# EDIpack/EDIpack

Measured on AMD Instinct MI355X. Metric: Lanczos H*v iterations/sec, largest (Nup,Ndw) sector, higher is better.
Workload: dtype f64

## Files before the change

edipack_amd/capi.py:

```python
from __future__ import annotations

import ctypes as C
import os

import numpy as np

HERE = os.path.dirname(os.path.abspath(__file__))
LIB_PATH = os.environ.get("EDIGPU_LIB", os.path.join(HERE, "lib", "libedigpu.so"))
HEADER_PATH = os.path.join(os.path.dirname(HERE), "include", "edigpu.h")

MAXORB = 5
MAXSUNDRY = 64
MAXBATH = 16


class EdigpuError(RuntimeError):
    """Raised when a C-ABI call returns non-zero (the Fortran shim does ``stop msg``)."""


class EdigpuModel(C.Structure):
    _fields_ = [
        ("ed_mode", C.c_int32), ("bath_type", C.c_int32),
        ("norb", C.c_int32), ("nbath", C.c_int32), ("nspin", C.c_int32), ("hfmode", C.c_int32),
        ("xmu", C.c_double),
# ... 90 lines not shown
    "edigpu_imp_rdm": (C.c_int, [_vp, _vp, C.c_int, _pd, _pd]),
    "edigpu_time_rdm": (C.c_int, [_vp, _vp, C.c_int, C.c_int, _pd]),
    "edigpu_imp_rdm_flat": (C.c_int, [_vp, _vp, C.c_int, _pd, _pd]),
    "edigpu_time_rdm_flat": (C.c_int, [_vp, _vp, C.c_int, C.c_int, _pd]),
    "edigpu_apply_xph": (C.c_int, [_vp, _vp, _vp, _vp]),
    "edigpu_ph_rdm": (C.c_int, [_vp, _vp, C.c_int, _pd, _pd]),
    "edigpu_time_ph": (C.c_int, [_vp, _vp, _vp, C.c_int, C.c_int, _pd]),
    "edigpu_pairs_sector": (C.c_int, [C.POINTER(EdigpuModel), C.c_int, C.c_int, C.c_int, _pi32, _pi32, _pi32, _pi32, _pi32,
                                      _pi32, _pint, _pint, _pint]),
    "edigpu_apply_pairs_normal": (C.c_int, [_vp, _vp, _vp, _vp, C.c_int, _pd, _pi32, _pi32, _pi32, _pi32, _pi32, _pi32, _vp]),
    "edigpu_time_pairs": (C.c_int, [_vp, _vp, _vp, _vp, C.c_int, _pd, _pi32, _pi32, _pi32, _pi32, _pi32, _pi32, C.c_int,
                                    C.c_int, _pd]),
    "edigpu_vec_work_doubles": (C.c_int, []),
    "edigpu_vec_rotate": (C.c_int, [_i64, _vp, _vp, _vp, _vp]),
    "edigpu_vec_add_dot": (C.c_int, [_i64, _vp, _vp, _vp, _vp, _vp, _vp]),
    "edigpu_vec_axpy_nrm2": (C.c_int, [_i64, _vp, _vp, _vp, _vp, _vp, _vp]),
    "edigpu_vec_scale": (C.c_int, [_i64, _vp, _vp, _vp]),
    "edigpu_vec_rotate_lazy": (C.c_int, [_i64, _vp, _vp, _vp, _vp]),
    "edigpu_vec_add_dot2": (C.c_int, [_i64, _vp, _vp, _vp, _vp, _vp, _vp]),
    "edigpu_time_apply": (C.c_int, [_vp, C.c_int, C.c_int, C.c_int, _pd]),
    "edigpu_lanczos_bench": (C.c_int, [_vp, C.c_int, C.c_int, _pd, _pd]),
    "edigpu_apply_loop_d": (C.c_int, [_vp, _i64, _pd, _pd]),
    "edigpu_tile_task_map": (C.c_int, [C.c_int32, C.c_int32, C.c_int32, _pi32, _pi32, _pi32, _pi32, _pi32]),
    "edigpu_ell16_images": (C.c_int, [_i64, _pi64, _pi32, _pd, _pi64, _vp, _vp, _pi64]),
    "edigpu_finalize_ab": (C.c_int, [C.c_int32, _pd, _i64, _pd, _pd, C.c_int32, _pd, C.c_int32, C.c_int32]),
    "edigpu_trl_dots": (C.c_int, [C.c_int32, _i64, C.c_int32, _pd, C.c_int32, _i64, _i64, _pd, _i64, C.c_int32, _pd, _i64,
                                  C.c_int32]),
    "edigpu_trl_norm2": (C.c_int, [C.c_int32, _i64, _pd, _i64, _pd, _i64]),
    "edigpu_trl_subtract": (C.c_int, [C.c_int32, _i64, C.c_int32, _pd, C.c_int32, _i64, _i64, _pd, _i64, _pd, _i64,
                                      C.c_int32]),
    "edigpu_trl_decide": (C.c_int, [_pd, _i64, C.c_int32, C.c_double, C.c_double, _pd, _i64, _pi32]),
    "edigpu_trl_filter": (C.c_int, [_pd, _i64, C.c_int32, C.c_double]),
    "edigpu_trl_rotate": (C.c_int, [_i64, C.c_int32, C.c_int32, _pd, _i64, _i64, _pd, C.c_int32, _i64, _pd, _i64, _i64]),
    "edigpu_trl_scale": (C.c_int, [_i64, _pd, _i64, C.c_double]),
    "edigpu_membw": (C.c_int, [_i64, _pd]),
    "edigpu_sector_map": (C.c_int, [_vp, C.c_int, C.c_int, C.c_int, _pi32, _pi64]),
    "edigpu_cache_create": (C.c_int, [C.POINTER(_vp), _i64]),
    "edigpu_cache_get": (C.c_int, [_vp, C.POINTER(EdigpuModel), C.c_int, C.c_int, C.c_int, C.POINTER(_vp)]),
    "edigpu_cache_stats": (C.c_int, [_vp, _pi64]),
    "edigpu_cache_clear": (C.c_int, [_vp]),
    "edigpu_cache_destroy": (C.c_int, [_vp]),
    "edigpu_dev_alloc": (C.c_int, [_i64, C.POINTER(_vp)]),
    "edigpu_dev_free": (C.c_int, [_vp]),
    "edigpu_dev_upload": (C.c_int, [_vp, _vp, _i64]),
    "edigpu_dev_download": (C.c_int, [_vp, _vp, _i64]),
    "edigpu_shard_plan": (C.c_int, [_i64, C.c_int32, C.c_int32, _pi64, _pi64, _pi64]),
# ... 90 lines not shown
```

edipack_amd/csrc/edigpu_capi.hip:

```cpp
#include <algorithm>
#include <map>
#include <mutex>
#include <tuple>

#include "dev_mem.hpp"
#include "host_ib.hpp"
#include "kernels.hpp"

namespace edigpu {

static thread_local std::string g_err;
static thread_local int g_device = 0;
void set_error(const std::string& msg) { g_err = msg; }

bool have_error() { return !g_err.empty(); }
int current_device() { return g_device; }

int ensure_device(int* count_out) {
  int n = 0;
  hipError_t e = hipGetDeviceCount(&n);
  if (e != hipSuccess || n <= 0) {
    set_error(std::string("edigpu: no usable HIP device (") +
              (e != hipSuccess ? hipGetErrorString(e) : "device count 0") +
              "); this library has no CPU fallback");
// ... 242 lines not shown
  if (bytes > 0) EDIGPU_HIP(hipMemcpy(dst_dev, src_host, (size_t)bytes, hipMemcpyHostToDevice));
  return 0;
}

int edigpu_dev_download(void* dst_host, const void* src_dev, int64_t bytes) {
  if (bytes < 0 || (bytes > 0 && (!dst_host || !src_dev))) {
    set_error("edigpu_dev_download: bad argument");
    return 1;
  }
  if (bytes > 0) EDIGPU_HIP(hipMemcpy(dst_host, src_dev, (size_t)bytes, hipMemcpyDeviceToHost));
  return 0;
}

int edigpu_destroy(edigpu_handle s) {
  if (!s) return 0;
  (void)hipSetDevice(s->device);
  if (s->stream) {
    (void)hipStreamSynchronize(s->stream);
    (void)hipStreamDestroy(s->stream);
  }
  if (s->sub_s) edigpu_destroy(s->sub_s);
  if (s->sub_a) edigpu_destroy(s->sub_a);
  if (s->sub_d) edigpu_destroy(s->sub_d);
  dev_free_all(s->d_cz, s->d_hd, s->d_gu, s->d_gd, s->d_mx_rowptr, s->d_tile_chunks, s->d_tile_lbeg);
  if (s->lz_graph) (void)hipGraphExecDestroy(s->lz_graph);
  dev_free_all(s->d_lzcnt, s->d_bl_meta, s->d_bl_lend, s->d_bl_ent, s->d_bl_wtab);
  if (s->ib) {
    free_ib(s->ib);
    delete s->ib;
    s->ib = nullptr;
  }
  dev_free_all(s->d_tl_meta, s->d_tl_col, s->d_tl_val, s->d_mx_col, s->d_mx_val);
  dev_free_all(s->d_eux, s->d_ed, s->d_impd, s->d_ndcoef, s->d_jup, s->d_jdw);
  free_ell(s->up_ell);
  free_csr(s->dw);
  free_csr(s->nd);
  free_csr(s->loc);
  free_csr(s->nonloc);
  dev_free_all(s->orbs.ell_col, s->orbs.ell_val, s->orbs.hd, s->orbs.eax, s->orbs.impbit, s->orbs.xtab);
  s->orbs = OrbsArgs();
  dev_free_all(s->d_dir_states, s->d_dir_offdw, s->d_dir_rkup, s->d_dir_terms, s->d_dir_tests, s->d_dir_dtab, s->d_dir_xtab);
  free_occ(s);
  free_rdm(s);
  free_rdm_flat(s);
  free_ph(s);
  free_axisop(s);
  free_batch(s);
// ... 7 lines not shown
```

edipack_amd/csrc/edigpu_internal.hpp:

```cpp
#pragma once
#include <hip/hip_runtime.h>

#include <cstdint>
#include <cstdio>
#include <functional>
#include <memory>
#include <string>
#include <vector>

#include "../../include/edigpu.h"
#include "host_build.hpp"
#include "switches.hpp"

namespace edigpu {

enum SectorKind : int { kNormal = 0, kFlat = 1, kDirect = 2, kOrbs = 3, kCmplxNormal = 4 };

void set_error(const std::string& msg);
#pragma GCC visibility push(hidden)
bool have_error();
int current_device();
int ensure_device(int* count_out = nullptr);
#pragma GCC visibility pop

// ... 178 lines not shown
  double* d_hd = nullptr;
  edigpu::DevEll up_ell;
  edigpu::DevCsr dw;
  int dw_maxrow = 0;
  edigpu::DevCsr nd;
  int has_nd = 0;
  edigpu::HostCsr h_up, h_dw;
  int rows_per_block = 1;
  int factored = 0;
  int fac_nimp = 0, fac_nterms = 0;
  double* d_eux = nullptr;
  double* d_ed = nullptr;
  uint8_t* d_impd = nullptr;
  double* d_ndcoef = nullptr;
  uint32_t* d_jup = nullptr;
  edigpu_sector* sub_s = nullptr;
  edigpu_sector* sub_a = nullptr;
  edigpu_sector* sub_d = nullptr;
  double* d_cz = nullptr;
  int panel_mode = 0;
  int tile_nchunks = 0, tile_rows = 0;
  int32_t* d_tile_chunks = nullptr;
  int32_t* d_tile_lbeg = nullptr;
  int tile_list_cap = 0;
  int4* d_tl_meta = nullptr;
  int32_t* d_tl_col = nullptr;
  double* d_tl_val = nullptr;
  int tl_has_nd = 0;
  int blk_shift = 0;
  int blk_tail_balance = 1;
  int64_t blk_ps = 0, blk_len = 0;
  int4* d_bl_meta = nullptr;
  int blk_rows = 0;
  int blk_list_cap = 0;
  int32_t* d_bl_lend = nullptr;
  uint32_t* d_bl_ent = nullptr;
  double* d_bl_wtab = nullptr;
  bool lz_blocked = false;
  int64_t lz_len = 0;
  edigpu::IbDev* ib = nullptr;
  int row_split = 1;
  int col_halo = 0;
  uint32_t* d_jdw = nullptr;
  int32_t* d_mx_rowptr = nullptr;
  int32_t* d_mx_col = nullptr;
  double* d_mx_val = nullptr;
// ... 97 lines not shown
```

edipack_amd/csrc/edigpu_setup.hip:

```cpp
#include <algorithm>
#include <cstddef>
#include <memory>

#include "dev_mem.hpp"
#include "host_ib.hpp"
#include "host_pack.hpp"
#include "host_sb.hpp"
#include "kernels.hpp"

namespace edigpu {

static const int4* as_int4(const std::vector<HostInt4>& v) {
  static_assert(sizeof(HostInt4) == sizeof(int4) && offsetof(HostInt4, x) == offsetof(int4, x) &&
                    offsetof(HostInt4, y) == offsetof(int4, y) && offsetof(HostInt4, z) == offsetof(int4, z) &&
                    offsetof(HostInt4, w) == offsetof(int4, w),
                "HostInt4 is uploaded as int4");
  return reinterpret_cast<const int4*>(v.data());
}

static int upload_csr(DevCsr& d, int64_t nrow, const int64_t* rowptr, const int32_t* col,
                      const double* val, int cplx) {
  d = DevCsr();
  d.nrow = nrow;
  d.nnz = rowptr ? rowptr[nrow] : 0;
// ... 398 lines not shown
        if (dev_upload(&s->d_mx_rowptr, m.rowptr.data(), m.rowptr.size()) || dev_upload(&s->d_mx_col, m.col.data(), m.col.size()) ||
            dev_upload(&s->d_mx_val, m.val.data(), m.val.size()))
          return 1;
      }
    }
    s->h_hd = std::move(built->hd);
    s->h_nd = std::move(built->nd);
  } else {
    if (dev_upload(&s->d_hd, hd, (size_t)s->nloc)) return 1;
    if (s->has_nd && upload_csr(s->nd, s->nloc, nd_rowptr, nd_col, nd_val, 0)) return 1;
    if (s->has_nd && !sw.nd_in_rows &&
        upload_sell(s->nd, s->nloc, dim_up * dim_dw, nd_rowptr, nd_col, nd_val, 0, false, sw, 16.0))
      return 1;
  }
  if (s->panel_mode == 2) {
    const HostFactored* f = (s->factored && built) ? &built->fac : nullptr;
    const bool with_nd = f && f->nterms > 0 && s->d_mx_rowptr != nullptr;
    const HostTileLists l = build_tile_lists(dw, dim_dw, dw_first, dw_count, tile_starts, with_nd ? f : nullptr);
    s->tile_list_cap = l.list_cap;
    const std::vector<HostInt4> meta = tile_meta_live(l, dw_first);
    if (dev_upload(&s->d_tile_lbeg, l.lbeg.data(), l.lbeg.size()) || dev_upload(&s->d_tl_meta, as_int4(meta), meta.size()) ||
        dev_upload(&s->d_tl_col, l.col.data(), l.col.size()) || dev_upload(&s->d_tl_val, l.val.data(), l.val.size()))
      return 1;
    s->tl_has_nd = l.has_nd ? 1 : 0;
  }
  if (s->factored && built && built->norb > 0 && dw_first == 0 && dw_count == dim_dw) {
    const int64_t min_rows = sw.ib_min;
    bool pairs = false;
    for (int sp = 0; sp < 2 && !pairs; sp++) {
      const std::vector<double>& a = built->ob_a[sp];
      const int ns = built->ns;
      if ((int)a.size() == ns * ns)
        for (int p = built->norb; p < ns && !pairs; p++)
          for (int q = p + 1; q < ns; q++)
            if (a[(size_t)p * ns + q] != 0.0) {
              pairs = true;
              break;
            }
    }
    const bool pairs_ok = !pairs || min_rows == 0 || sw.ib_pairs;
    const bool short_rows = dim_up * 8 < sw.ib_min_row_bytes();
    if (sw.ib && pairs_ok && s->nloc >= min_rows && (!short_rows || sw.posrows) && !sw.lanczos_unfused && setup_ib(s, *built))
      return 1;
    if (s->ib && short_rows && !s->ib->pr.on) {
      free_ib(s->ib);
      delete s->ib;
// ... 244 lines not shown
```

edipack_amd/csrc/hooks/image_hooks.hip:

```cpp
#include <algorithm>
#include <climits>

#include "../dev_mem.hpp"
#include "../host_pack.hpp"
#include "../kernels.hpp"
#include "../tile_map.hpp"

using namespace edigpu;

extern "C" {

int edigpu_tile_task_map(int32_t npanels, int32_t blocks_per_panel, int32_t balanced, int32_t* grid, int32_t* np,
                         int32_t* panel, int32_t* chunk, int32_t* pos) {
  if (npanels < 1 || blocks_per_panel < 1 || !grid || !np ||
      ((int64_t)npanels + 7) / 8 * 8 * (int64_t)blocks_per_panel > INT32_MAX) {
    set_error("edigpu_tile_task_map: bad argument");
    return 1;
  }
  const TileMap m = plan_tile_map(npanels, blocks_per_panel, balanced != 0);
  *grid = m.grid;
  *np = m.np;
  for (int wg = 0; wg < m.grid; wg++) {
    int pn, ch, ps;
    if (!tile_task_of(m, npanels, blocks_per_panel, wg, pn, ch, ps)) pn = -1;
    if (panel) panel[wg] = pn;
    if (chunk) chunk[wg] = ch;
    if (pos) pos[wg] = ps;
  }
  return 0;
}

int edigpu_ell16_images(int64_t nrow, const int64_t* rowptr, const int32_t* col, const double* val, int64_t* info,
                        uint32_t* pk16, uint32_t* pk16o, int64_t* owned_col) {
  if (nrow < 1 || !rowptr || !info || (rowptr[nrow] > 0 && (!col || !val))) {
    set_error("edigpu_ell16_images: bad argument");
    return 1;
  }
  HostCsr a;
  a.nrow = a.ncol = nrow;
  a.rowptr.assign(rowptr, rowptr + nrow + 1);
  a.col.assign(col, col + rowptr[nrow]);
  a.val.assign(val, val + rowptr[nrow]);
  const HostEll h = encode_ell(a, true, true, true);
  info[0] = h.width;
  info[1] = h.pitch;
  info[2] = h.pitch16o;
  info[3] = (int64_t)h.pk16.size();
  info[4] = (int64_t)h.pk16o.size();
  if (pk16) std::copy(h.pk16.begin(), h.pk16.end(), pk16);
  if (pk16o) std::copy(h.pk16o.begin(), h.pk16o.end(), pk16o);
  if (owned_col)
// ... 31 lines not shown
```

edipack_amd/csrc/host_pack.cpp:

```cpp
#include "host_pack.hpp"

#include <algorithm>
#include <cmath>
#include <cstdlib>
#include <cstring>

namespace edigpu {

HostEll encode_ell(const HostCsr& a, bool lds, bool allow_typed, bool allow_16) {
  HostEll e;
  const uint32_t cmul = lds ? 8u : 1u;
  e.nrow = a.nrow;
  e.pitch = (a.nrow + 63) / 64 * 64;
  int w = 0;
  for (int64_t i = 0; i < a.nrow; i++) w = std::max<int>(w, (int)(a.rowptr[i + 1] - a.rowptr[i]));
  e.width = w;
  if (w == 0 || a.nrow == 0) return e;
  std::vector<double> coef(1, 0.0);
  bool packable = (a.nrow + 1) * (int64_t)cmul < ((int64_t)1 << 24);
  std::vector<uint8_t> cid((size_t)a.nnz());
  for (int64_t p = 0; p < a.nnz() && packable; p++) {
    const double m = std::fabs(a.val[p]);
    size_t k = 0;
    for (; k < coef.size(); k++)
// ... 302 lines not shown
  }
  for (size_t ch = 0; ch + 1 < tile_starts.size(); ch++) lbeg.push_back(meta[(size_t)tile_starts[ch]].x);
  lbeg.push_back((int32_t)tc.size());
  l.list_cap = 4;
  for (size_t ch = 0; ch + 1 < lbeg.size(); ch++) l.list_cap = std::max(l.list_cap, lbeg[ch + 1] - lbeg[ch]);
  tc.resize(tc.size() + 8, 0);
  tv.resize(tv.size() + 8, 0.0);
  l.has_nd = with_nd;
  return l;
}

std::vector<HostInt4> tile_meta_live(const HostTileLists& l, int64_t dw_first) {
  std::vector<HostInt4> meta = l.meta;
  for (size_t r = 0; r < meta.size(); r++) {
    HostInt4& m = meta[r];
    const int ob = m.x + m.y;
    while (m.z % 4 != 1 && m.z > 0 && l.val[(size_t)(ob + m.z - 1)] == 0.0 &&
           l.col[(size_t)(ob + m.z - 1)] == (int32_t)(dw_first + (int64_t)r))
      m.z--;
  }
  return meta;
}

HostBlockLists build_block_lists(const HostCsr& dw, const HostFactored& f, int64_t dim_dw, int shift, int64_t lds_kb) {
  HostBlockLists b;
  std::vector<double> wtab{0.0};
  auto widx = [&](double w) -> int {
    for (size_t i = 0; i < wtab.size(); i++)
      if (wtab[i] == w && std::signbit(wtab[i]) == std::signbit(w)) return (int)i;
    wtab.push_back(w);
    return (int)wtab.size() - 1;
  };
  int64_t R = std::max<int64_t>(32, std::min<int64_t>(lds_kb * 1024 / ((int64_t)8 << shift), 4096) / 32 * 32);
  std::vector<HostInt4> meta((size_t)dim_dw);
  std::vector<uint32_t> ent;
  ent.reserve((size_t)dw.rowptr[dim_dw] + 8 * (size_t)dim_dw);
  bool fits = true;
  for (int64_t g = 0; g < dim_dw && fits; g++) {
    const int64_t cs = g / R * R;
    HostInt4 m = {(int)ent.size(), 0, 0, 0};
    for (int pass = 0; pass < 2; pass++) {
      int& cnt = pass == 0 ? m.y : m.z;
      for (int64_t q = dw.rowptr[g]; q < dw.rowptr[g + 1]; q++) {
        const int64_t c = dw.col[q];
        const bool inside = c >= cs && c < cs + R;
        if (inside != (pass == 0)) continue;
// ... 51 lines not shown
```

edipack_amd/csrc/host_pack.hpp:

```cpp
#pragma once
#include <cstdint>
#include <vector>

#include "host_build.hpp"

namespace edigpu {

struct HostInt4 {
  int32_t x, y, z, w;
};

struct HostEll {
  int64_t nrow = 0, pitch = 0;
  int width = 0;
  int typed = 0;
  std::vector<uint32_t> pk;
  std::vector<double> coef;
  std::vector<uint32_t> pk16;
  std::vector<uint32_t> pk16o;
  int64_t pitch16o = 0;
  std::vector<int32_t> col;
  std::vector<double> val;
};
inline int64_t ell16_owned_col(int64_t pos) {
// ... 16 lines not shown
                     bool is_loc, double max_pad, bool allow_packed);

void plan_tile_chunks(const HostCsr& dw, int64_t dw_first, int64_t dw_count, int rmax, std::vector<int32_t>& starts,
                      int& longest);

struct HostMergedList {
  std::vector<int32_t> rowptr, col;
  std::vector<double> val;
};
HostMergedList merge_dw_lists(const HostCsr& dw, const HostFactored& f, int64_t dw_first, int64_t dw_count, int64_t dim_dw);

struct HostTileLists {
  std::vector<HostInt4> meta;
  std::vector<int32_t> col;
  std::vector<double> val;
  std::vector<int32_t> lbeg;
  int list_cap = 4;
  bool has_nd = false;
};
HostTileLists build_tile_lists(const HostCsr& dw, int64_t dim_dw, int64_t dw_first, int64_t dw_count,
                               const std::vector<int32_t>& tile_starts, const HostFactored* f);
std::vector<HostInt4> tile_meta_live(const HostTileLists& l, int64_t dw_first);

struct HostBlockLists {
  bool fits = false;
  int rows = 0;
  std::vector<HostInt4> meta;
  std::vector<uint32_t> ent;
  std::vector<double> wtab;
  std::vector<int32_t> lend;
  int list_cap = 4;
};
HostBlockLists build_block_lists(const HostCsr& dw, const HostFactored& f, int64_t dim_dw, int shift, int64_t lds_kb);

int factored_col_halo(const HostFactored& f, int64_t dim_up);

}
```

edipack_amd/csrc/kernels_normal.hip:

```cpp
#include <cstdlib>
#include <string>
#include <type_traits>

#include "kernels.hpp"
#include "normal_args.hpp"

namespace edigpu {



constexpr int kE = 4;

template <bool VEC>
__device__ inline void load4(const double* __restrict__ base, int64_t i0, const bool* ok, double* out, int64_t dB = 2) {
  if (VEC) {
    const double2 a = ok[0] ? *reinterpret_cast<const double2*>(base + i0) : make_double2(0.0, 0.0);
    const double2 b = ok[2] ? *reinterpret_cast<const double2*>(base + i0 + dB) : make_double2(0.0, 0.0);
    out[0] = a.x;
    out[1] = a.y;
    out[2] = b.x;
    out[3] = b.y;
  } else {
#pragma unroll
    for (int e = 0; e < kE; e++) out[e] = ok[e] ? base[i0 + e] : 0.0;
// ... 522 lines not shown
  a.ell_val = s->up_ell.val;
  a.ell_w = s->up_ell.width;
  a.ell_typed = s->up_ell.typed;
  a.ell_pitch = s->up_ell.pitch;
  a.ell_pitch16 = s->up_ell.pitch16;
  a.dw_rowptr = s->dw.rowptr32;
  a.dw_col = s->dw.col;
  a.dw_val = s->dw.val;
  a.dw_maxrow = s->dw_maxrow;
  a.nd_rp32 = s->nd.rowptr32;
  a.nd_rp64 = s->nd.wide ? s->nd.rowptr64 : nullptr;
  a.nd_col = s->nd.col;
  a.nd_val = s->nd.val;
  a.has_nd = s->has_nd;
  a.nterms = s->factored ? s->fac_nterms : 0;
  a.nd_coef = s->d_ndcoef;
  a.jup = s->d_jup;
  a.jdw = s->d_jdw;
  a.panel_mode = s->panel_mode;
  a.tile_nchunks = s->tile_nchunks;
  a.tile_rows = s->tile_rows;
  a.tile_chunks = s->d_tile_chunks;
  a.tile_lbeg = s->d_tile_lbeg;
  a.tile_list_cap = s->tile_list_cap;
  a.tl_meta = s->d_tl_meta;
  a.tl_col = s->d_tl_col;
  a.tl_val = s->d_tl_val;
  a.tl_has_nd = s->tl_has_nd;
  a.blk_shift = 0;
  a.blk_ps = 0;
  a.blk_tail_balance = s->blk_tail_balance;
  a.bl_meta = s->d_bl_meta;
  a.blk_rows = s->blk_rows;
  a.blk_list_cap = s->blk_list_cap;
  a.bl_lend = s->d_bl_lend;
  a.bl_ent = s->d_bl_ent;
  a.bl_wtab = s->d_bl_wtab;
  a.mx_rowptr = s->d_mx_rowptr;
  a.mx_col = s->d_mx_col;
  a.mx_val = s->d_mx_val;
  a.scal = nullptr;
  a.partial = nullptr;
  a.xout = nullptr;
  a.partial_cap = 0;
  a.lz_counter = nullptr;
  a.lz_nlanc = 0;
// ... 146 lines not shown
```

edipack_amd/csrc/kernels_panel.hip:

```cpp
#include <algorithm>
#include <cstdio>
#include <cstdlib>
#include <vector>

#include "lz_finalize.hpp"
#include "normal_args.hpp"
#include "tile_map.hpp"

namespace edigpu {

struct PanelArgs {
  int npanels, width, blocks_per_panel, rows_per_block;
  int64_t col_first, ncol, stride;
  int halo;
  int tile_rows;
  int list_cap;
  TileMap map;
};

constexpr int kPanelNT = 512;
constexpr int kMaxNdTerms = 16;

template <bool DO_DW, bool DO_ND, bool ALPHA, bool COLS = false>
__global__ void __launch_bounds__(kPanelNT)
    normal_dw_panel_kernel(NormalArgs a, PanelArgs p, const double* __restrict__ v_full,
                           double* __restrict__ hv) {
  __shared__ double red[3 * (kPanelNT / 64)];
// ... 314 lines not shown
    if (threadIdx.x == 0) {
#pragma unroll
      for (int i = 0; i < kPanelNT / 64; i++) {
        t += red[i];
        q += red[kPanelNT / 64 + i];
        n += red[2 * (kPanelNT / 64) + i];
      }
      if (!a.lz_counter) {
        a.partial[blockIdx.x] = t;
        a.partial[gridDim.x + blockIdx.x] = q;
        a.partial[2 * gridDim.x + blockIdx.x] = n;
      }
    }
    if (a.lz_counter)
      lz_finalize_if_last<kPanelNT>(a.lz_counter, a.partial, t, q, n, v_full, hv, a.lz_len, const_cast<double*>(a.scal),
                                    a.lz_nlanc, lzsh);
  }
}

constexpr int kTileSeg = 64;
constexpr int kTileRowsPerWave = 4;
constexpr int kTileMaxRows = kTileRowsPerWave * 16;
constexpr int kTileBatch = 4;

template <int NT, bool DO_ND, bool ALPHA, bool EDGE, bool BLK = false>
__global__ void __launch_bounds__(NT)
    normal_dw_tile_kernel(NormalArgs a, PanelArgs p, const double* __restrict__ v_full, double* __restrict__ hv) {
  __shared__ double red[3 * (NT / 64)];
  extern __shared__ double2 tile[];
  double* lval = reinterpret_cast<double*>(tile + (size_t)p.tile_rows * kTileSeg);
  int32_t* lcol = reinterpret_cast<int32_t*>(lval + p.list_cap);
  int4* lmeta = reinterpret_cast<int4*>(lcol + p.list_cap);
  uint32_t* ju2 = reinterpret_cast<uint32_t*>(lmeta + p.tile_rows);
  const int x = blockIdx.x & 7, slot = blockIdx.x >> 3, nslots = gridDim.x >> 3;
  int bpanel = 0, bchunk = 0, ppos = blockIdx.x;
  const int np = BLK ? p.map.np : (int)gridDim.x;
  const bool has_task = !BLK || tile_task_of(p.map, p.npanels, p.blocks_per_panel, blockIdx.x, bpanel, bchunk, ppos);
  if (ALPHA && BLK && (int)blockIdx.x >= p.map.wg_tail && bpanel == p.map.panel_tail && threadIdx.x < 24) {
    const int xx = threadIdx.x & 7;
    if (p.map.panel_tail + xx >= p.npanels) a.partial[(threadIdx.x >> 3) * np + ppos + xx] = 0.0;
  }
  if (ALPHA && a.scal[SC_STOP] != 0.0) {
    if (threadIdx.x == 0) {
      a.partial[ppos] = 0.0;
      a.partial[np + ppos] = 0.0;
      a.partial[2 * np + ppos] = 0.0;
    }
    return;
  }
  double asum = 0.0, qsum = 0.0, nsum = 0.0;
  const double sg = ALPHA ? a.scal[SC_ALPHA] : 0.0;
  const int lane = threadIdx.x & 63;
  const int wave = __builtin_amdgcn_readfirstlane(threadIdx.x >> 6);
  constexpr int NW = NT / 64;
  const int64_t DimUp = a.dim_up;
  int cur_panel = -1;
  for (int task = slot, it = 0;; task += nslots, it++) {
    if (BLK && (it > 0 || !has_task)) break;
    const int panel = BLK ? bpanel : (task / p.blocks_per_panel) * 8 + x;
    if (panel >= p.npanels) break;
    const int chunk = BLK ? bchunk : task % p.blocks_per_panel;
    const int rb = a.tile_chunks[chunk], nrows = a.tile_chunks[chunk + 1] - rb;
    const int lb = a.tile_lbeg[chunk], ln = a.tile_lbeg[chunk + 1] - lb;
    const int64_t pbase = (int64_t)panel * p.width;
    const int64_t RS = BLK ? 128 : DimUp;
    const double* __restrict__ vb = BLK ? v_full + (int64_t)panel * a.blk_ps : v_full;
    double* __restrict__ hb = BLK ? hv + (int64_t)panel * a.blk_ps : hv;
    auto col_of = [&](int l, bool& okl, bool& pairl) -> int64_t {
      const int64_t cl = pbase + 2 * l;
      okl = 2 * l < p.width && cl < DimUp;
      const int64_t ccl = okl ? cl : (EDGE ? DimUp - 1 : DimUp - 2);
      pairl = !EDGE || ccl + 1 < DimUp;
      return ccl;
    };
    bool ok, pair;
    int64_t cc = col_of(lane, ok, pair);
    int64_t c = pbase + 2 * lane;
    if (BLK) {
      cc = c = 2 * lane;
      ok = pair = true;
    }
    auto ld2 = [&](const double* q) -> double2 {
      if (!EDGE) return *reinterpret_cast<const double2*>(q);
      if (pair) {
        const d2u t = *reinterpret_cast<const d2u*>(q);
        return make_double2(t.x, t.y);
      }
      return make_double2(q[0], 0.0);
    };
    auto st2 = [&](double* q, double2 t) {
      if (!EDGE) {
        *reinterpret_cast<double2*>(q) = t;
      } else if (pair) {
        d2u u;
        u.x = t.x;
        u.y = t.y;
        *reinterpret_cast<d2u*>(q) = u;
      } else {
        q[0] = t.x;
      }
    };
    const int64_t g0 = a.dw_first + rb;
    double2 acc[kTileRowsPerWave];
    {
      double2 own[kTileRowsPerWave];
#pragma unroll
      for (int j = 0; j < kTileRowsPerWave; j++) {
        const int r = wave + j * NW;
        const int rr = r < nrows ? r : nrows - 1;
        acc[j] = ld2(&hb[(int64_t)(rb + rr) * RS + cc]);
      }
#pragma unroll
      for (int j = 0; j < kTileRowsPerWave; j++) {
        const int r = wave + j * NW;
        const int rr = r < nrows ? r : nrows - 1;
        own[j] = ld2(&vb[(g0 + rr) * RS + cc]);
      }
      for (int i = threadIdx.x; i < ln; i += NT) {
        lcol[i] = a.tl_col[lb + i];
        lval[i] = a.tl_val[lb + i];
      }
      if ((int)threadIdx.x < nrows) {
        int4 m = a.tl_meta[rb + threadIdx.x];
        m.x -= lb;
        lmeta[threadIdx.x] = m;
      }
#pragma unroll
      for (int j = 0; j < kTileRowsPerWave; j++) {
        const int r = wave + j * NW;
        const int rr = r < nrows ? r : nrows - 1;
        tile[rr * kTileSeg + lane] = own[j];
// ... 107 lines not shown
            p1 = trow[j1 & 127u];
          } else {
            const double2 y = ld2(&vb[prow * RS + cc]);
            const int l0 = (int)((j0 >> 1) & 63u), l1 = (int)((j1 >> 1) & 63u);
            const double s0x = __shfl(y.x, l0, 64), s0y = __shfl(y.y, l0, 64);
            const double s1x = __shfl(y.x, l1, 64), s1y = __shfl(y.y, l1, 64);
            p0 = (j0 & 1u) ? s0y : s0x;
            p1 = (j1 & 1u) ? s1y : s1x;
          }
          auto edge = [&](uint32_t jw) -> double {
            const int64_t jc = (int64_t)(jw & 0x3FFFFFFFu);
            return BLK ? v_full[(jc >> 7) * a.blk_ps + prow * 128 + (jc & 127)] : v_full[prow * DimUp + jc];
          };
          if (v0 && (j0 & 0x40000000u)) p0 = edge(j0);
          if (v1 && (j1 & 0x40000000u)) p1 = edge(j1);
          s.x += w0 * p0;
          s.y += w1 * p1;
        }
      }
      return s;
    };
#pragma unroll
    for (int j = 0; j < kTileRowsPerWave; j++) {
      const int r = wave + j * NW;
      if (r < nrows) {
        acc[j] = row_sum(r, acc[j]);
        if (ok) {
          st2(&hb[(int64_t)(rb + r) * RS + c], acc[j]);
          if (ALPHA) {
            const double2 o = tile[r * kTileSeg + lane];
            const double dx = acc[j].x - sg * o.x, dy = acc[j].y - sg * o.y;
            asum += o.x * acc[j].x + o.y * acc[j].y;
            qsum += dx * dx + dy * dy;
            nsum += o.x * o.x + o.y * o.y;
          }
        }
      }
    }
    __syncthreads();
  }
  if (ALPHA) {
#pragma unroll
    for (int off = 32; off > 0; off >>= 1) {
      asum += __shfl_down(asum, off, 64);
      qsum += __shfl_down(qsum, off, 64);
      nsum += __shfl_down(nsum, off, 64);
    }
// ... 240 lines not shown
    __syncthreads();
    double t = 0.0, q = 0.0, n = 0.0;
    if (threadIdx.x == 0) {
#pragma unroll
      for (int i = 0; i < NW; i++) {
        t += red[i];
        q += red[NW + i];
        n += red[2 * NW + i];
      }
      if (!a.lz_counter) {
        a.partial[blockIdx.x] = t;
        a.partial[gridDim.x + blockIdx.x] = q;
        a.partial[2 * gridDim.x + blockIdx.x] = n;
      }
    }
    if (a.lz_counter)
      lz_finalize_if_last<kBlkNT>(a.lz_counter, a.partial, t, q, n, v, hv, a.lz_len, const_cast<double*>(a.scal), a.lz_nlanc,
                                  lzsh);
  }
}

static int launch_dw_blocked_tiles(const NormalArgs& a, bool do_nd, const double* v, double* hv, hipStream_t st, bool alpha,
                                   int* nblocks) {
  if (!a.tile_chunks || !a.tl_meta || a.tile_rows > kTileMaxRows || (do_nd && !a.tl_has_nd) || a.dw_first != 0 ||
      a.dw_count != a.dim_dw) {
    set_error("launch_dw_blocked: 128-column panels need the tiled sweep's row lists");
    return 1;
  }
  PanelArgs p;
  p.width = 128;
  p.npanels = (int)((a.dim_up + 127) / 128);
  p.col_first = 0;
  p.ncol = a.dim_up;
  p.stride = a.dim_up;
  p.halo = 0;
  p.rows_per_block = 0;
  p.tile_rows = a.tile_rows;
  p.blocks_per_panel = a.tile_nchunks;
  p.list_cap = a.tile_list_cap;
  const int panel_groups = (p.npanels + 7) / 8;
  const int64_t np = (int64_t)panel_groups * p.blocks_per_panel * 8;
  if (np > INT32_MAX || (alpha && 3 * np > a.partial_cap)) {
    set_error("launch_dw_blocked: partial buffer too small for this grid");
    return 1;
  }
  p.map = plan_tile_map(p.npanels, p.blocks_per_panel, a.blk_tail_balance != 0 && !a.lz_counter);
  const int g = p.map.grid;
// ... 125 lines not shown
  p.rows_per_block = (int)((a.dw_count + bpp - 1) / bpp);
  if (p.rows_per_block < 16) p.rows_per_block = 16;
  bpp = (int)((a.dw_count + p.rows_per_block - 1) / p.rows_per_block);
  p.blocks_per_panel = bpp;
  const int panel_groups = (p.npanels + 7) / 8;
  const dim3 grid((unsigned)((int64_t)panel_groups * bpp * 8)), block(kPanelNT);
  if (do_nd)
    hipLaunchKernelGGL((normal_dw_panel_kernel<true, true, false, true>), grid, block, 0, st, a, p, w, hv);
  else
    hipLaunchKernelGGL((normal_dw_panel_kernel<true, false, false, true>), grid, block, 0, st, a, p, w, hv);
  EDIGPU_HIP(hipGetLastError());
  return 0;
}

int launch_dw_panels(const NormalArgs& a, const Switches& sw, bool do_dw, bool do_nd, const double* v_full, double* hv,
                     hipStream_t st, bool alpha, int* nblocks) {
  if (!do_dw && !do_nd && !alpha) return 0;
  if (do_nd && a.nterms > kMaxNdTerms) {
    set_error("launch_dw_panels: too many factored Hnd terms");
    return 1;
  }
  const bool edge = (a.dim_up % 2) != 0;
  const bool vec2 = a.panel_mode >= 1 && do_dw && (((uintptr_t)v_full | (uintptr_t)hv) & (edge ? 7 : 15)) == 0;
  const bool tiled = vec2 && a.panel_mode == 2 && a.tile_chunks != nullptr && a.tl_meta != nullptr && a.tile_rows <= kTileMaxRows &&
                     (!do_nd || a.tl_has_nd);
  PanelArgs p;
  if (vec2) {
    int wmax = sw.panel_w.value_or(128) & ~1;
    if (wmax < 2 || wmax > 128) wmax = 128;
    int np = (int)((a.dim_up + 8 * wmax - 1) / (8 * wmax)) * 8;
    if (np < 8) np = 8;
    p.width = (int)((a.dim_up + np - 1) / np);
    p.width += p.width & 1;
    p.npanels = (int)((a.dim_up + p.width - 1) / p.width);
  } else {
    plan_panels(p, a.dim_up, sw);
  }
  p.col_first = 0;
  p.ncol = a.dim_up;
  p.stride = a.dim_up;
  p.halo = 0;
  p.tile_rows = 0;
  int bpp = panel_resident_blocks(sw);
  if (vec2 && !sw.panel_bpp) bpp = 256;
  p.rows_per_block = (int)((a.dw_count + bpp - 1) / bpp);
  if (p.rows_per_block < 16) p.rows_per_block = 16;
  bpp = (int)((a.dw_count + p.rows_per_block - 1) / p.rows_per_block);
// ... 96 lines not shown
```

edipack_amd/csrc/normal_args.hpp:

```cpp
#pragma once
#include <cstdint>

#include "kernels.hpp"

namespace edigpu {

struct NormalArgs {
  int64_t dim_up, dim_dw, dw_first, dw_count;
  const double* hd;
  const double* eux;
  const double* ed;
  const uint8_t* impd;
  const uint32_t* ell_pk;
  const double* ell_coef;
  const uint32_t* ell_pk16;
  const int32_t* ell_col;
  const double* ell_val;
  int ell_w;
  int ell_typed;
  int64_t split_first, split_count;
  int64_t ell_pitch;
  int64_t ell_pitch16;
  const int32_t* dw_rowptr;
  const int32_t* dw_col;
  const double* dw_val;
  const int32_t* nd_rp32;
  const int64_t* nd_rp64;
  const int32_t* nd_col;
  const double* nd_val;
  int dw_maxrow;
  int has_nd;
  int nterms;
  const double* nd_coef;
  const uint32_t* jup;
  const uint32_t* jdw;
  const double* scal;
  double* partial;
  double* xout;
  int64_t partial_cap;
  unsigned int* lz_counter;
  int lz_nlanc;
  int64_t lz_len;
  int panel_mode;
  int tile_nchunks, tile_rows;
  const int32_t* tile_chunks;
  const int32_t* tile_lbeg;
  int tile_list_cap;
  const int4* tl_meta;
  const int32_t* tl_col;
  const double* tl_val;
  int tl_has_nd;
  int blk_shift;
  int blk_tail_balance;
  int64_t blk_ps;
  const int4* bl_meta;
  const uint32_t* bl_ent;
  int blk_rows;
  int blk_list_cap;
  const int32_t* bl_lend;
  const double* bl_wtab;
  const int32_t* mx_rowptr;
  const int32_t* mx_col;
  const double* mx_val;
};

int launch_dw_panels(const NormalArgs& a, const Switches& sw, bool do_dw, bool do_nd, const double* v_full, double* hv,
                     hipStream_t st, bool alpha = false, int* nblocks = nullptr);

int launch_dw_blocked(const NormalArgs& a, const Switches& sw, bool do_nd, const double* v, double* hv, hipStream_t st, bool alpha,
                      int* nblocks);
// ... 6 lines not shown
```

edipack_amd/csrc/switches.hpp:

```cpp
#pragma once
#include <cstdint>
#include <limits>
#include <optional>

namespace edigpu {

enum class SwitchRule {
  Present,
  FirstIsOne,
  OnUnlessZero,
  OffUnlessNonzero,
  Int,
  Int64,
  IntOrUnset,
  Int64OrUnset,
  DoubleOrUnset,
};
enum class SwitchMoment { SetUp, Comm, Loop };

struct SwitchRow {
  const char* name;
  SwitchRule rule;
  int64_t dflt, lo, hi;
  SwitchMoment moment;
// ... 9 lines not shown
#define EDIGPU_SETUP_SWITCHES(X)                                                                                                            \
                                                                                                         \
  X(ell16, bool, "EDIGPU_ELL16", OnUnlessZero, 1, 0, 1, "0: no 16-bit LDS image of Hup beside the packed one")                              \
  X(ell_untyped, bool, "EDIGPU_ELL_UNTYPED", Present, 0, 0, 1, "Hup as plain ELL (column, value), not the packed typed image")            \
  X(csr_nosell, bool, "EDIGPU_CSR_NOSELL", Present, 0, 0, 1, "stored sectors stay CSR: no SELL-64 image")                                  \
  X(csr_unpacked, bool, "EDIGPU_CSR_UNPACKED", Present, 0, 0, 1, "SELL-64 image with explicit values, not the value dictionary")          \
  X(normal_explicit, bool, "EDIGPU_NORMAL_EXPLICIT", FirstIsOne, 0, 0, 1, "normal mode: explicit diagonal and Hnd, not the factored tables") \
  X(handover_factor, bool, "EDIGPU_HANDOVER_FACTOR", OnUnlessZero, 1, 0, 1, "0: handed-over arrays are not searched for the factored form") \
  X(nd_in_rows, bool, "EDIGPU_ND_IN_ROWS", FirstIsOne, 0, 0, 1, "explicit Hnd as CSR inside the row kernel, not as its own SELL pass")     \
  X(nd_no_merge, bool, "EDIGPU_ND_NO_MERGE", Present, 0, 0, 1, "factored Hnd terms of equal partner maps are not merged")                  \
  X(cmplx_fourproducts, bool, "EDIGPU_CMPLX_FOURPRODUCTS", FirstIsOne, 0, 0, 1, "complex normal mode as four real products, not the doubled real sector") \
  X(flat_hostbuild, bool, "EDIGPU_FLAT_HOSTBUILD", FirstIsOne, 0, 0, 1, "stored superc / nonsu2 image built on the host, not on the device") \
  X(direct_nosort, bool, "EDIGPU_DIRECT_NOSORT", Present, 0, 0, 1, "on-the-fly terms keep the builder's order")                            \
  X(direct_termorder, bool, "EDIGPU_DIRECT_TERMORDER", Present, 0, 0, 1, "on-the-fly kernel walks all terms, no per-workgroup compaction") \
  X(direct_wgs, int, "EDIGPU_DIRECT_WGS", Int, 2, -kSwAny, kSwAny, "on-the-fly kernel: persistent workgroups per CU")                      \
                                                                      \
  X(rows_td, OptInt, "EDIGPU_ROWS_TD", IntOrUnset, 0, 0, 0, "rows per workgroup of the LDS row kernel (1, 2, 4, 8); unset: from the row length") \
  X(row_split, OptInt, "EDIGPU_ROW_SPLIT", IntOrUnset, 0, 0, 0, "column parts long rows are staged in (0: never); unset: as many as the LDS needs") \
  X(panel_vec2, bool, "EDIGPU_PANEL_VEC2", OnUnlessZero, 1, 0, 1, "0: no two-column panel sweep")                                          \
  X(panel_vec2_min, int64_t, "EDIGPU_PANEL_VEC2_MIN", Int64, (int64_t)1 << 21, -kSwAny, kSwAny, "smallest sector (rows) of the two-column and tiled sweeps") \
  X(panel_tile, bool, "EDIGPU_PANEL_TILE", OnUnlessZero, 1, 0, 1, "0: no LDS-tiled panel sweep")                                           \
  X(tile_rows, int, "EDIGPU_TILE_ROWS", Int, 32, 8, 64, "rows of a chunk of the tiled sweep")                                               \
  X(tile_balance, bool, "EDIGPU_TILE_BALANCE", OnUnlessZero, 1, 0, 1, "0: padded grid of the tiled sweep, last panel group not spread over the XCDs") \
  X(tile_persist, bool, "EDIGPU_TILE_PERSIST", OffUnlessNonzero, 0, 0, 1, "tiled sweep as a persistent grid")                              \
  X(panel_w, OptInt, "EDIGPU_PANEL_W", IntOrUnset, 0, 0, 0, "widest panel (columns); unset or out of range: 64, two-column sweep 128")      \
  X(panel_bpp, OptInt, "EDIGPU_PANEL_BPP", IntOrUnset, 0, 0, 0, "workgroups per panel; unset: 128, two-column sweep 256")                   \
  X(blocked, bool, "EDIGPU_BLOCKED", OnUnlessZero, 1, 0, 1, "0: the Lanczos loop keeps the natural vector layout")                         \
  X(blocked_min, int64_t, "EDIGPU_BLOCKED_MIN", Int64, (int64_t)1 << 21, -kSwAny, kSwAny, "smallest sector (rows) of the panel-major loop") \
  X(blocked_w, int, "EDIGPU_BLOCKED_W", Int, 128, -kSwAny, kSwAny, "panel width of that loop: 128 (tiled sweep), 64 / 32 / 16 (narrow-panel sweep); else none") \
  X(blocked_lds_kb, int64_t, "EDIGPU_BLOCKED_LDS_KB", Int64, 32, -kSwAny, kSwAny, "KiB of staged segments per block of the narrow-panel sweep") \
  X(blocked_wgs, int, "EDIGPU_BLOCKED_WGS", Int, 8, -kSwAny, kSwAny, "narrow-panel sweep: workgroups per CU (1 .. 8, else 8)")             \
                                                                                                                  \
  X(ib, bool, "EDIGPU_IB", OnUnlessZero, 1, 0, 1, "0: no impurity-block image")                                                            \
  X(ib_min, int64_t, "EDIGPU_IB_MIN", Int64, (int64_t)1 << 21, -kSwAny, kSwAny, "smallest sector (elements) that gets it; 0 also lifts the row and pair gates") \
  X(ib_minrow, OptInt64, "EDIGPU_IB_MINROW", Int64OrUnset, 0, 0, 0, "shortest row (bytes) on its rows kernels; unset: 40960, or 0 when EDIGPU_IB_MIN=0") \
  X(ib_rows, int, "EDIGPU_IB_ROWS", Int, 480, 4, 480, "rows of a staged chunk of its columns kernel")                                       \
  X(ib_pairs, bool, "EDIGPU_IB_PAIRS", FirstIsOne, 0, 0, 1, "replica / general baths take the image too")                                  \
  X(ib_split, OptInt, "EDIGPU_IB_SPLIT", IntOrUnset, 0, 0, 0, "rows staged in halves: non-zero always, 0 never; unset: rows longer than the LDS") \
  X(ib_nsub, int, "EDIGPU_IB_NSUB", Int, 1, 1, 8, "workgroups per chunk of the columns kernel")                                            \
  X(ib_pspad, int, "EDIGPU_IB_PSPAD", Int, 0, 0, kSwAny, "doubles between two panels (rounded down to even)")                              \
  X(ib_nt, int, "EDIGPU_IB_NT", Int, 0, -kSwAny, kSwAny, "threads per workgroup of the rows kernel; 0: the best that fits")                \
  X(ib_cols2, OptInt, "EDIGPU_IB_COLS2", IntOrUnset, 0, 0, 0, "pipelined columns kernel: non-zero on, 0 off; unset: panels above 2 MiB")   \
  X(ib_verbose, bool, "EDIGPU_IB_VERBOSE", Present, 0, 0, 1, "say on stderr why a sector gets no image")                                   \
  X(posrows, bool, "EDIGPU_POSROWS", OffUnlessNonzero, 0, 0, 1, "short rows: the generic LDS row kernel in position order beside the block columns kernel") \
                                                                                                      \
  X(sb, bool, "EDIGPU_SB", OnUnlessZero, 1, 0, 1, "0: the impurity-block kernels, no local-block tables")                                  \
// ... 49 lines not shown
```

include/edigpu.h:

```cpp
#ifndef EDIGPU_H
#define EDIGPU_H

#include <stdint.h>

#ifdef __cplusplus
extern "C" {
#endif

#define EDIGPU_MAXORB 5
#define EDIGPU_MAXSUNDRY 64
#define EDIGPU_MAXBATH 16

typedef struct edigpu_sector *edigpu_handle;

const char *edigpu_last_error(void);
int edigpu_version(void);
int64_t edigpu_model_sizeof(void);
int edigpu_device_count(int *count);
int edigpu_init(int device);

int edigpu_normal_create(edigpu_handle *h, int64_t dim_up, int64_t dim_dw, int64_t dw_first,
                         int64_t dw_count, const double *hd, const int64_t *up_rowptr,
                         const int32_t *up_col, const double *up_val, const int64_t *dw_rowptr,
                         const int32_t *dw_col, const double *dw_val, const int64_t *nd_rowptr,
// ... 186 lines not shown
                                double *eval, double *evec_shard, int *nmatvec);
int edigpu_apply_cops_sharded(edigpu_handle src, edigpu_handle dst, edigpu_comm c, const double *v_src_shard,
                              double *v_dst_shard, int nops, const double *coef_re_im, const int32_t *create,
                              const int32_t *iorb, const int32_t *ispin);
int edigpu_lanczos_bench_sharded(edigpu_handle h, edigpu_comm c, int warmup, int steps, double *ms_per_step,
                                 int64_t *exchange_bytes);

int edigpu_exchange_bench(edigpu_handle h, edigpu_comm c, int steps, int32_t *rccl_ranks, double *ms_exchange);

typedef struct edigpu_cache_s *edigpu_cache;
int edigpu_cache_create(edigpu_cache *c, int64_t max_device_bytes);
int edigpu_cache_get(edigpu_cache c, const edigpu_model *model, int kind, int q1, int q2, edigpu_handle *h);
int edigpu_cache_stats(edigpu_cache c, int64_t stats[5]);
int edigpu_cache_clear(edigpu_cache c);
int edigpu_cache_destroy(edigpu_cache c);

int edigpu_time_apply(edigpu_handle h, int warmup, int steps, int lanczos, double *ms_per_step);

int edigpu_apply_loop_d(edigpu_handle h, int64_t nloc, const double *v_host, double *hv_host);

int edigpu_tile_task_map(int32_t npanels, int32_t blocks_per_panel, int32_t balanced, int32_t *grid, int32_t *np,
                         int32_t *panel, int32_t *chunk, int32_t *pos);

int edigpu_ell16_images(int64_t nrow, const int64_t *rowptr, const int32_t *col, const double *val, int64_t *info,
                        uint32_t *pk16, uint32_t *pk16o, int64_t *owned_col);

int edigpu_finalize_ab(int32_t np, const double *partial, int64_t n, const double *P, const double *Q, int32_t nscal,
                       double *scal, int32_t iter, int32_t nlanc);

int edigpu_trl_dots(int32_t cplx, int64_t n, int32_t ndot, const double *Q, int32_t ncol, int64_t ldq, int64_t qlen,
                    const double *w, int64_t wlen, int32_t w_col, double *h, int64_t hlen, int32_t skip);
int edigpu_trl_norm2(int32_t cplx, int64_t n, const double *w, int64_t wlen, double *h, int64_t hlen);
int edigpu_trl_subtract(int32_t cplx, int64_t n, int32_t nvec, const double *Q, int32_t ncol, int64_t ldq, int64_t qlen,
                        const double *h, int64_t hlen, double *w, int64_t wlen, int32_t skip);
int edigpu_trl_decide(const double *h, int64_t hlen, int32_t nvec, double eta2, double thr2, double *hf, int64_t hflen,
                      int32_t *skip);
int edigpu_trl_filter(double *h, int64_t hlen, int32_t nvec, double thr2);
int edigpu_trl_rotate(int64_t len, int32_t m, int32_t k, const double *Q, int64_t ldq, int64_t qlen, const double *Y,
                      int32_t ldy, int64_t ylen, double *out, int64_t ldo, int64_t olen);
int edigpu_trl_scale(int64_t len, double *v, int64_t vlen, double f);

int edigpu_lanczos_bench(edigpu_handle h, int warmup, int steps, double *ms_wall_per_step,
                         double *ms_hv_per_launch);

int edigpu_dev_alloc(int64_t bytes, void **dev_ptr);
int edigpu_dev_free(void *dev_ptr);
// ... 12 lines not shown
```

Baseline: 7451.

## Assign tiled-sweep chunk rows to waves by modelled cost instead of round-robin

Adds a host-built per-chunk row map that packs four row indices per wave into a uint32. Rows are greedily assigned, longest first, to the least-loaded wave using a cost model built from list lengths and nd terms. The map is used only when its worst wave load does not exceed the round-robin one. The tiled panel kernel now reads row indices from this map rather than computing wave + j*NW, which aims to cut wave imbalance inside a chunk. The cost is one extra global load per wave and some setup work; the tiled path now also requires the map to be present.

Result: no change. 7473, median of 6 (+0.3%).

```diff
diff --git a/edipack_amd/capi.py b/edipack_amd/capi.py
--- a/edipack_amd/capi.py
+++ b/edipack_amd/capi.py
@@ -136,6 +136,8 @@
     "edigpu_lanczos_bench": (C.c_int, [_vp, C.c_int, C.c_int, _pd, _pd]),
     "edigpu_apply_loop_d": (C.c_int, [_vp, _i64, _pd, _pd]),
     "edigpu_tile_task_map": (C.c_int, [C.c_int32, C.c_int32, C.c_int32, _pi32, _pi32, _pi32, _pi32, _pi32]),
+    "edigpu_tile_rowmap": (C.c_int, [_i64, _vp, _vp, _vp, C.c_int32, _vp, _vp, _i64, _i64, C.c_int32, C.c_int32, _vp, _vp, _vp, _vp,
+                                     _vp]),
     "edigpu_ell16_images": (C.c_int, [_i64, _pi64, _pi32, _pd, _pi64, _vp, _vp, _pi64]),
     "edigpu_finalize_ab": (C.c_int, [C.c_int32, _pd, _i64, _pd, _pd, C.c_int32, _pd, C.c_int32, C.c_int32]),
     "edigpu_trl_dots": (C.c_int, [C.c_int32, _i64, C.c_int32, _pd, C.c_int32, _i64, _i64, _pd, _i64, C.c_int32, _pd, _i64,
diff --git a/edipack_amd/csrc/edigpu_capi.hip b/edipack_amd/csrc/edigpu_capi.hip
--- a/edipack_amd/csrc/edigpu_capi.hip
+++ b/edipack_amd/csrc/edigpu_capi.hip
@@ -288,7 +288,7 @@
   if (s->sub_s) edigpu_destroy(s->sub_s);
   if (s->sub_a) edigpu_destroy(s->sub_a);
   if (s->sub_d) edigpu_destroy(s->sub_d);
-  dev_free_all(s->d_cz, s->d_hd, s->d_gu, s->d_gd, s->d_mx_rowptr, s->d_tile_chunks, s->d_tile_lbeg);
+  dev_free_all(s->d_cz, s->d_hd, s->d_gu, s->d_gd, s->d_mx_rowptr, s->d_tile_chunks, s->d_tile_lbeg, s->d_tile_rowmap);
   if (s->lz_graph) (void)hipGraphExecDestroy(s->lz_graph);
   dev_free_all(s->d_lzcnt, s->d_bl_meta, s->d_bl_lend, s->d_bl_ent, s->d_bl_wtab);
   if (s->ib) {
diff --git a/edipack_amd/csrc/edigpu_internal.hpp b/edipack_amd/csrc/edigpu_internal.hpp
--- a/edipack_amd/csrc/edigpu_internal.hpp
+++ b/edipack_amd/csrc/edigpu_internal.hpp
@@ -224,6 +224,7 @@
   int tile_nchunks = 0, tile_rows = 0;
   int32_t* d_tile_chunks = nullptr;
   int32_t* d_tile_lbeg = nullptr;
+  uint32_t* d_tile_rowmap = nullptr;
   int tile_list_cap = 0;
   int4* d_tl_meta = nullptr;
   int32_t* d_tl_col = nullptr;
diff --git a/edipack_amd/csrc/edigpu_setup.hip b/edipack_amd/csrc/edigpu_setup.hip
--- a/edipack_amd/csrc/edigpu_setup.hip
+++ b/edipack_amd/csrc/edigpu_setup.hip
@@ -444,6 +444,8 @@
     if (dev_upload(&s->d_tile_lbeg, l.lbeg.data(), l.lbeg.size()) || dev_upload(&s->d_tl_meta, as_int4(meta), meta.size()) ||
         dev_upload(&s->d_tl_col, l.col.data(), l.col.size()) || dev_upload(&s->d_tl_val, l.val.data(), l.val.size()))
       return 1;
+    const std::vector<uint32_t> rowmap = build_tile_rowmap(tile_starts, meta, tile_map_waves(s->tile_rows), sw.tile_rowmap);
+    if (dev_upload(&s->d_tile_rowmap, rowmap.data(), rowmap.size())) return 1;
     s->tl_has_nd = l.has_nd ? 1 : 0;
   }
   if (s->factored && built && built->norb > 0 && dw_first == 0 && dw_count == dim_dw) {
diff --git a/edipack_amd/csrc/hooks/image_hooks.hip b/edipack_amd/csrc/hooks/image_hooks.hip
--- a/edipack_amd/csrc/hooks/image_hooks.hip
+++ b/edipack_amd/csrc/hooks/image_hooks.hip
@@ -27,6 +27,46 @@
     if (chunk) chunk[wg] = ch;
     if (pos) pos[wg] = ps;
   }
+  return 0;
+}
+
+int edigpu_tile_rowmap(int64_t dim_dw, const int64_t* rowptr, const int32_t* col, const double* val, int32_t nterms,
+                       const double* coef, const uint32_t* jdw, int64_t dw_first, int64_t dw_count, int32_t rmax, int32_t by_cost,
+                       int32_t* info, int32_t* starts, int32_t* meta, int32_t* cost, uint32_t* map) {
+  if (dim_dw < 1 || !rowptr || (rowptr[dim_dw] > 0 && (!col || !val)) || nterms < 0 || (nterms > 0 && (!coef || !jdw)) ||
+      dw_first < 0 || dw_count < 1 || dw_first + dw_count > dim_dw || rmax < 8 || rmax > 64 || !info || !starts || !meta ||
+      !cost || !map) {
+    set_error("edigpu_tile_rowmap: bad argument");
+    return 1;
+  }
+  HostCsr dw;
+  dw.nrow = dw.ncol = dim_dw;
+  dw.rowptr.assign(rowptr, rowptr + dim_dw + 1);
+  dw.col.assign(col, col + rowptr[dim_dw]);
+  dw.val.assign(val, val + rowptr[dim_dw]);
+  HostFactored f;
+  f.valid = true;
+  f.nterms = nterms;
+  if (nterms > 0) {
+    f.coef.assign(coef, coef + nterms);
+    f.jdw.assign(jdw, jdw + (size_t)nterms * dim_dw);
+  }
+  std::vector<int32_t> st;
+  int longest = 0;
+  plan_tile_chunks(dw, dw_first, dw_count, rmax, st, longest);
+  const HostTileLists l = build_tile_lists(dw, dim_dw, dw_first, dw_count, st, nterms > 0 ? &f : nullptr);
+  const std::vector<HostInt4> live = tile_meta_live(l, dw_first);
+  const int nw = tile_map_waves(longest);
+  const std::vector<uint32_t> m = build_tile_rowmap(st, live, nw, by_cost != 0);
+  const int32_t v[8] = {(int32_t)st.size() - 1, nw, kTileCostTrip, kTileCostFixed, kTileCostInside, kTileCostNd, longest, 0};
+  std::copy(v, v + 8, info);
+  std::copy(st.begin(), st.end(), starts);
+  for (size_t r = 0; r < live.size(); r++) {
+    const int32_t q[4] = {live[r].x, live[r].y, live[r].z, live[r].w};
+    std::copy(q, q + 4, meta + 4 * r);
+    cost[r] = tile_row_cost(live[r]);
+  }
+  std::copy(m.begin(), m.end(), map);
   return 0;
 }
 
diff --git a/edipack_amd/csrc/host_pack.cpp b/edipack_amd/csrc/host_pack.cpp
--- a/edipack_amd/csrc/host_pack.cpp
+++ b/edipack_amd/csrc/host_pack.cpp
@@ -348,6 +348,47 @@
   return meta;
 }
 
+std::vector<uint32_t> build_tile_rowmap(const std::vector<int32_t>& tile_starts, const std::vector<HostInt4>& live_meta, int nw,
+                                        bool by_cost) {
+  const size_t nchunks = tile_starts.empty() ? 0 : tile_starts.size() - 1;
+  std::vector<uint32_t> map(nchunks * (size_t)nw, 0xFFFFFFFFu);
+  std::vector<int> order, load((size_t)nw), cnt((size_t)nw);
+  std::vector<uint32_t> word((size_t)nw);
+  for (size_t ch = 0; ch < nchunks; ch++) {
+    const int cs = tile_starts[ch], n = tile_starts[ch + 1] - cs;
+    uint32_t* w = &map[ch * (size_t)nw];
+    if (n > nw * kTileMapRowsPerWave) continue;
+    int rr_longest = 0;
+    for (int wv = 0; wv < nw; wv++) {
+      int chain = 0;
+      for (int j = 0, r = wv; j < kTileMapRowsPerWave && r < n; j++, r += nw) {
+        w[wv] = (w[wv] & ~(0xFFu << (8 * j))) | ((uint32_t)r << (8 * j));
+        chain += tile_row_cost(live_meta[(size_t)(cs + r)]);
+      }
+      rr_longest = std::max(rr_longest, chain);
+    }
+    if (!by_cost) continue;
+    order.resize((size_t)n);
+    for (int r = 0; r < n; r++) order[(size_t)r] = r;
+    std::stable_sort(order.begin(), order.end(), [&](int a, int b) {
+      return tile_row_cost(live_meta[(size_t)(cs + a)]) > tile_row_cost(live_meta[(size_t)(cs + b)]);
+    });
+    std::fill(load.begin(), load.end(), 0);
+    std::fill(cnt.begin(), cnt.end(), 0);
+    std::fill(word.begin(), word.end(), 0xFFFFFFFFu);
+    for (const int r : order) {
+      int best = -1;
+      for (int wv = 0; wv < nw; wv++)
+        if (cnt[(size_t)wv] < kTileMapRowsPerWave && (best < 0 || load[(size_t)wv] < load[(size_t)best])) best = wv;
+      const int j = cnt[(size_t)best]++;
+      load[(size_t)best] += tile_row_cost(live_meta[(size_t)(cs + r)]);
+      word[(size_t)best] = (word[(size_t)best] & ~(0xFFu << (8 * j))) | ((uint32_t)r << (8 * j));
+    }
+    if (*std::max_element(load.begin(), load.end()) <= rr_longest) std::copy(word.begin(), word.end(), w);
+  }
+  return map;
+}
+
 HostBlockLists build_block_lists(const HostCsr& dw, const HostFactored& f, int64_t dim_dw, int shift, int64_t lds_kb) {
   HostBlockLists b;
   std::vector<double> wtab{0.0};
diff --git a/edipack_amd/csrc/host_pack.hpp b/edipack_amd/csrc/host_pack.hpp
--- a/edipack_amd/csrc/host_pack.hpp
+++ b/edipack_amd/csrc/host_pack.hpp
@@ -62,6 +62,15 @@
                                const std::vector<int32_t>& tile_starts, const HostFactored* f);
 std::vector<HostInt4> tile_meta_live(const HostTileLists& l, int64_t dw_first);
 
+constexpr int kTileMapRowsPerWave = 4;
+inline int tile_map_waves(int longest_chunk) { return longest_chunk > 8 * kTileMapRowsPerWave ? 16 : 8; }
+constexpr int kTileCostTrip = 20, kTileCostFixed = 6, kTileCostInside = 2, kTileCostNd = 3;
+inline int tile_row_cost(const HostInt4& live_meta) {
+  return kTileCostTrip * ((live_meta.z + 3) / 4) + kTileCostFixed + kTileCostInside * (live_meta.y / 4) + kTileCostNd * live_meta.w;
+}
+std::vector<uint32_t> build_tile_rowmap(const std::vector<int32_t>& tile_starts, const std::vector<HostInt4>& live_meta, int nw,
+                                        bool by_cost);
+
 struct HostBlockLists {
   bool fits = false;
   int rows = 0;
diff --git a/edipack_amd/csrc/kernels_normal.hip b/edipack_amd/csrc/kernels_normal.hip
--- a/edipack_amd/csrc/kernels_normal.hip
+++ b/edipack_amd/csrc/kernels_normal.hip
@@ -568,6 +568,7 @@
   a.tile_rows = s->tile_rows;
   a.tile_chunks = s->d_tile_chunks;
   a.tile_lbeg = s->d_tile_lbeg;
+  a.tile_rowmap = s->d_tile_rowmap;
   a.tile_list_cap = s->tile_list_cap;
   a.tl_meta = s->d_tl_meta;
   a.tl_col = s->d_tl_col;
diff --git a/edipack_amd/csrc/kernels_panel.hip b/edipack_amd/csrc/kernels_panel.hip
--- a/edipack_amd/csrc/kernels_panel.hip
+++ b/edipack_amd/csrc/kernels_panel.hip
@@ -3,6 +3,7 @@
 #include <cstdlib>
 #include <vector>
 
+#include "host_pack.hpp"
 #include "lz_finalize.hpp"
 #include "normal_args.hpp"
 #include "tile_map.hpp"
@@ -363,6 +364,8 @@
 constexpr int kTileRowsPerWave = 4;
 constexpr int kTileMaxRows = kTileRowsPerWave * 16;
 constexpr int kTileBatch = 4;
+static_assert(kTileRowsPerWave == kTileMapRowsPerWave && kTileRowsPerWave * (kPanelNT / 64) == 8 * kTileMapRowsPerWave,
+              "the row map (host_pack.hpp) is built for this geometry: tile_map_waves() waves of four rows");
 
 template <int NT, bool DO_ND, bool ALPHA, bool EDGE, bool BLK = false>
 __global__ void __launch_bounds__(NT)
@@ -403,6 +406,8 @@
     const int chunk = BLK ? bchunk : task % p.blocks_per_panel;
     const int rb = a.tile_chunks[chunk], nrows = a.tile_chunks[chunk + 1] - rb;
     const int lb = a.tile_lbeg[chunk], ln = a.tile_lbeg[chunk + 1] - lb;
+    const uint32_t rmap = a.tile_rowmap[chunk * NW + wave];
+    auto row_of = [&](int j) -> int { return (int)((rmap >> (8 * j)) & 0xFFu); };
     const int64_t pbase = (int64_t)panel * p.width;
     const int64_t RS = BLK ? 128 : DimUp;
     const double* __restrict__ vb = BLK ? v_full + (int64_t)panel * a.blk_ps : v_full;
@@ -447,7 +452,7 @@
       double2 own[kTileRowsPerWave];
 #pragma unroll
       for (int j = 0; j < kTileRowsPerWave; j++) {
-        const int r = wave + j * NW;
+        const int r = row_of(j);
         const int rr = r < nrows ? r : nrows - 1;
         acc[j] = ld2(&hb[(int64_t)(rb + rr) * RS + cc]);
       }
@@ -601,7 +606,7 @@
     };
 #pragma unroll
     for (int j = 0; j < kTileRowsPerWave; j++) {
-      const int r = wave + j * NW;
+      const int r = row_of(j);
       if (r < nrows) {
         acc[j] = row_sum(r, acc[j]);
         if (ok) {
@@ -888,7 +893,7 @@
 
 static int launch_dw_blocked_tiles(const NormalArgs& a, bool do_nd, const double* v, double* hv, hipStream_t st, bool alpha,
                                    int* nblocks) {
-  if (!a.tile_chunks || !a.tl_meta || a.tile_rows > kTileMaxRows || (do_nd && !a.tl_has_nd) || a.dw_first != 0 ||
+  if (!a.tile_chunks || !a.tl_meta || !a.tile_rowmap || a.tile_rows > kTileMaxRows || (do_nd && !a.tl_has_nd) || a.dw_first != 0 ||
       a.dw_count != a.dim_dw) {
     set_error("launch_dw_blocked: 128-column panels need the tiled sweep's row lists");
     return 1;
@@ -1060,7 +1065,7 @@
   }
   const bool edge = (a.dim_up % 2) != 0;
   const bool vec2 = a.panel_mode >= 1 && do_dw && (((uintptr_t)v_full | (uintptr_t)hv) & (edge ? 7 : 15)) == 0;
-  const bool tiled = vec2 && a.panel_mode == 2 && a.tile_chunks != nullptr && a.tl_meta != nullptr && a.tile_rows <= kTileMaxRows &&
+  const bool tiled = vec2 && a.panel_mode == 2 && a.tile_chunks != nullptr && a.tl_meta != nullptr && a.tile_rowmap != nullptr && a.tile_rows <= kTileMaxRows &&
                      (!do_nd || a.tl_has_nd);
   PanelArgs p;
   if (vec2) {
diff --git a/edipack_amd/csrc/normal_args.hpp b/edipack_amd/csrc/normal_args.hpp
--- a/edipack_amd/csrc/normal_args.hpp
+++ b/edipack_amd/csrc/normal_args.hpp
@@ -46,6 +46,7 @@
   const int32_t* tile_chunks;
   const int32_t* tile_lbeg;
   int tile_list_cap;
+  const uint32_t* tile_rowmap;
   const int4* tl_meta;
   const int32_t* tl_col;
   const double* tl_val;
diff --git a/edipack_amd/csrc/switches.hpp b/edipack_amd/csrc/switches.hpp
--- a/edipack_amd/csrc/switches.hpp
+++ b/edipack_amd/csrc/switches.hpp
@@ -55,6 +55,7 @@
   X(panel_tile, bool, "EDIGPU_PANEL_TILE", OnUnlessZero, 1, 0, 1, "0: no LDS-tiled panel sweep")                                           \
   X(tile_rows, int, "EDIGPU_TILE_ROWS", Int, 32, 8, 64, "rows of a chunk of the tiled sweep")                                               \
   X(tile_balance, bool, "EDIGPU_TILE_BALANCE", OnUnlessZero, 1, 0, 1, "0: padded grid of the tiled sweep, last panel group not spread over the XCDs") \
+  X(tile_rowmap, bool, "EDIGPU_TILE_ROWMAP", OnUnlessZero, 1, 0, 1, "0: a chunk's rows go to the waves of the tiled sweep round-robin, not by modelled cost") \
   X(tile_persist, bool, "EDIGPU_TILE_PERSIST", OffUnlessNonzero, 0, 0, 1, "tiled sweep as a persistent grid")                              \
   X(panel_w, OptInt, "EDIGPU_PANEL_W", IntOrUnset, 0, 0, 0, "widest panel (columns); unset or out of range: 64, two-column sweep 128")      \
   X(panel_bpp, OptInt, "EDIGPU_PANEL_BPP", IntOrUnset, 0, 0, 0, "workgroups per panel; unset: 128, two-column sweep 256")                   \
diff --git a/include/edigpu.h b/include/edigpu.h
--- a/include/edigpu.h
+++ b/include/edigpu.h
@@ -232,6 +232,10 @@
 int edigpu_tile_task_map(int32_t npanels, int32_t blocks_per_panel, int32_t balanced, int32_t *grid, int32_t *np,
                          int32_t *panel, int32_t *chunk, int32_t *pos);
 
+int edigpu_tile_rowmap(int64_t dim_dw, const int64_t *rowptr, const int32_t *col, const double *val, int32_t nterms,
+                       const double *coef, const uint32_t *jdw, int64_t dw_first, int64_t dw_count, int32_t rmax,
+                       int32_t by_cost, int32_t *info, int32_t *starts, int32_t *meta, int32_t *cost, uint32_t *map);
+
 int edigpu_ell16_images(int64_t nrow, const int64_t *rowptr, const int32_t *col, const double *val, int64_t *info,
                         uint32_t *pk16, uint32_t *pk16o, int64_t *owned_col);
 
```
